# TU-Delft-AI-Energy-Lab/Deep-Statistical-Solver-for-Distribution-System-State-Estimation

Measured on AMD Instinct MI355X. Metric: grid-samples/sec fwd+bwd (WLS loss), CIGRE-14 batch=4096, 1/2/4/8 GPU, higher is better.
Workload: dtype f32 (H->H products as f16x3: two fp16 pieces per operand, 3 fp16 MFMAs per fp32 product, f32 accumulate; edge MLP bf16x6; everything else f32/f64); 1 GPU; CIGRE-14 (15 buses, 14 closed branches) B=4096 graphs/GPU, MPN L=4 H=128 K=2 dropout=0: forward + gsp_wls_edge + backward; graphs_per_gpu=4096, global_batch=4096, parallelism=dp1, ranks_seen=1, arithmetic_route=f16x3, plan_launches=9, clock_ramp_steps_before_warmup=5220, mode=launch plan (dss2_plan_run)

## Files before the change

### deep-statistical-solver-for-distribution-system-state-estimation_amd/csrc/dss2_wgrad16h.hip

```cpp
#include <stdlib.h>

#include "dss2_wgrad_batch.hpp"

namespace dss2 {

#ifdef DSS2_STAMPS
__device__ unsigned long long g_hstamps[512 * 4 * 16];
#define HSTAMP(slot)                                                                                   \
  do {                                                                                                 \
    if (stamp_on) {                                                                                    \
      unsigned long long t_;                                                                           \
      __builtin_amdgcn_sched_barrier(0);                                                               \
      asm volatile("s_memtime %0\n\ts_waitcnt lgkmcnt(0)" : "=s"(t_)::"memory");                      \
      __builtin_amdgcn_sched_barrier(0);                                                               \
      if (lane == 0 && blockIdx.x < 256 && blockIdx.z == 1) g_hstamps[((blockIdx.x * 2 + (blockIdx.y & 1)) * 4 + wv) * 16 + (slot)] = t_; \
    }                                                                                                  \
  } while (0)
#else
#define HSTAMP(slot) do {} while (0)
#endif

constexpr int W16H_TM = 32, W16H_ZC = 64, W16H_XW = 128, W16H_NT = 256, W16H_LDZF = 64, W16H_DMAX = 8;
__device__ __forceinline__ int tph_key(int col) { return (((col >> 3) & 1) << 1) | ((col >> 4) & 1); }
__device__ __forceinline__ int tph_off(int col, int row) { return col * 64 + ((((row >> 3) ^ tph_key(col)) << 4) | ((row & 7) << 1)); }

template <int NCOLS>
__device__ __forceinline__ void store_planes_h(char* img, int off0, const f32x4 v0, const f32x4 v1, int e) {
  const float s = pow2f(e);
#pragma unroll
  for (int q = 0; q < 4; ++q) {
    uint32_t h, l;
    split2_pair(v0[q] * s, v1[q] * s, h, l);
    char* dst = img + off0 + q * 64;
    *reinterpret_cast<uint32_t*>(dst) = h;
    *reinterpret_cast<uint32_t*>(dst + NCOLS * 64) = l;
  }
}

template <int NMAT, bool RS2>
__global__ void __launch_bounds__(W16H_NT, 2) wgrad16h_kernel(const dss2_wgrad_args p, int nibg, const WgradBatch wb, int hb) {
  constexpr int TM = W16H_TM, ZC = W16H_ZC, XW = W16H_XW, NT = W16H_NT, LDZF = W16H_LDZF;
  const float* __restrict__ Gp = wb.n > 0 ? wb.G[blockIdx.z] : p.G;
  const float* __restrict__ Xp = wb.n > 0 ? wb.X[blockIdx.z] : p.X;
  float* __restrict__ slabp = wb.n > 0 ? wb.slab[blockIdx.z] : p.slab;
  const float* __restrict__ rs2 = RS2 ? (wb.n > 0 ? wb.rowscale2[blockIdx.z] : p.rowscale2) : nullptr;
  extern __shared__ __attribute__((aligned(16))) float smem[];
  float* Zf0 = smem;
  float* Zf1 = Zf0 + TM * LDZF;
  char* ZT = reinterpret_cast<char*>(Zf1 + TM * LDZF);
  char* XT = ZT + NMAT * 2 * ZC * 64;
  int2* ell = reinterpret_cast<int2*>(XT + 2 * XW * 64);
  float* mxp = reinterpret_cast<float*>(ell + W16H_DMAX * TM);
  const int D = p.ell_width;

  const int tid = threadIdx.x;
  const int lane = tid & 63, c32 = lane & 31, half = lane >> 5;
  const int wv = __builtin_amdgcn_readfirstlane(tid >> 6);
  const int xb0 = 2 * (wv & 1), obw = wv >> 1;
  const int slice = blockIdx.x, ysl = blockIdx.y;
  const int obg = ysl / nibg, ibg = ysl - obg * nibg;
  const int gcol0 = obg * ZC, xcol0 = ibg * XW;
  const bool x_on[2] = {(xcol0 + xb0 * 32) < p.hin, (xcol0 + (xb0 + 1) * 32) < p.hin};
  const bool in_active = x_on[0] && (gcol0 + obw * 32) < p.hout;

  const int cg = tid & 15, rp = (tid >> 4) ^ ((tid & 1) << 1);
  const int g_off0 = tph_off(4 * cg, 2 * rp);
  const int x_off0[2] = {tph_off(4 * cg, 2 * rp), tph_off(64 + 4 * cg, 2 * rp)};
  const uint32_t g_goff = (uint32_t)((2 * rp) * p.ldg + 4 * cg) * 4u;

  f32x16 acc[2][NMAT];
#pragma unroll
  for (int xb = 0; xb < 2; ++xb)
#pragma unroll
    for (int m = 0; m < NMAT; ++m)
#pragma unroll
      for (int r = 0; r < 16; ++r) acc[xb][m][r] = 0.f;
  f32x4 bsum = {0.f, 0.f, 0.f, 0.f};
  f32x4 bs2[RS2 ? NMAT : 1];
#pragma unroll
  for (int m = 0; m < (RS2 ? NMAT : 1); ++m) bs2[m] = f32x4{0.f, 0.f, 0.f, 0.f};
  int Ex = -100, Eg = -100;

  typedef float f32x3 __attribute__((ext_vector_type(3)));
  f32x4 pg[2], px[4];
  f32x3 prs[RS2 ? 2 : 1];
  int2 pel;
  const uint32_t g_col = (gcol0 + 4 * cg < p.hout) ? (uint32_t)(4 * cg) * 4u : 0u;
  const bool g_ok = gcol0 + 4 * cg < p.hout;
  const uint32_t x_col[2] = {(xcol0 + 4 * cg < p.hin) ? (uint32_t)(4 * cg) * 4u : 0u, (xcol0 + 64 + 4 * cg < p.hin) ? (uint32_t)(64 + 4 * cg) * 4u : 0u};
  const float* __restrict__ rsb = RS2 ? (rs2 ? rs2 : Gp) : nullptr;
  auto load_tile = [&](int tile, int ts, int R) {
    const char* gb = reinterpret_cast<const char*>(Gp + (size_t)ts * p.ldg + gcol0);
    const char* xb = reinterpret_cast<const char*>(Xp + (size_t)ts * p.ldx + xcol0);
#pragma unroll
    for (int u = 0; u < 2; ++u) {
      const int r = 2 * rp + u;
      const int rr = r < R ? r : R - 1;
      pg[u] = *reinterpret_cast<const f32x4*>(gb + (uint32_t)(rr * p.ldg) * 4u + g_col);
      const uint32_t xro = (uint32_t)(rr * p.ldx) * 4u;
#ifdef DSS2_ABLATE_XLOAD
#pragma unroll
      for (int i = 0; i < 2; ++i) px[2 * i + u] = f32x4{1.f, 1.f, 1.f, 1.f};
      (void)xro; (void)xb;
#else
#pragma unroll
      for (int i = 0; i < 2; ++i) px[2 * i + u] = *reinterpret_cast<const f32x4*>(xb + xro + x_col[i]);
#endif
      if constexpr (RS2) prs[u] = *reinterpret_cast<const f32x3*>(rsb + (size_t)(ts + rr) * 4);
    }
    pel = tid < D * TM ? (reinterpret_cast<const int2*>(p.ell_tiles) + (size_t)tile * D * TM)[tid] : make_int2(tid & (TM - 1), 0);
  };
  auto publish_max = [&]() {
    float mx = 0.f, mg = 0.f;
#pragma unroll
    for (int i = 0; i < 4; ++i) mx = absmax4(mx, px[i]);
#pragma unroll
    for (int u = 0; u < 2; ++u) mg = absmax4(mg, pg[u]);
    mx = wave_max(mx); mg = wave_max(mg);
    if (lane == 0) { mxp[wv] = mx; mxp[4 + wv] = mg; }
  };
  auto prop = [&](const float* Zs, float* Zd, char* img, int ez) {
    f32x4 s[2];
#pragma unroll
    for (int u = 0; u < 2; ++u) {
      const int row = 2 * rp + u;
      f32x4 a = {0.f, 0.f, 0.f, 0.f};
      for (int k0 = 0; k0 < D; k0 += 4) {
        int2 en[4];
        f32x4 z[4];
#pragma unroll
        for (int k = 0; k < 4; ++k) en[k] = ell[(k0 + k) * TM + row];
#pragma unroll
        for (int k = 0; k < 4; ++k) z[k] = *reinterpret_cast<const f32x4*>(Zs + en[k].x * LDZF + 4 * cg);
#pragma unroll
        for (int k = 0; k < 4; ++k) {
          const float w = __int_as_float(en[k].y);
#pragma unroll
          for (int q = 0; q < 4; ++q) a[q] = fmaf(w, z[k][q], a[q]);
        }
      }
      s[u] = a;
      if (Zd) *reinterpret_cast<f32x4*>(Zd + row * LDZF + 4 * cg) = a;
    }
    store_planes_h<ZC>(img, g_off0, s[0], s[1], ez);
  };

  int ts = 0, R = 0, ts_n = 0, R_n = 0;
  if (slice < p.ntiles) {
    ts = p.tile_start[slice]; R = p.tile_start[slice + 1] - ts;
    load_tile(slice, ts, R);
    publish_max();
    if (slice + p.n_split < p.ntiles) { ts_n = p.tile_start[slice + p.n_split]; R_n = p.tile_start[slice + p.n_split + 1] - ts_n; }
  }
  __syncthreads();
  for (int tile = slice; tile < p.ntiles; tile += p.n_split) {
    const int next = tile + p.n_split;
#ifdef DSS2_STAMPS
    const bool stamp_on = tile == slice + 2 * p.n_split;
#endif
    HSTAMP(0);
    {
      const f32x4 m0 = *reinterpret_cast<const f32x4*>(mxp), m1 = *reinterpret_cast<const f32x4*>(mxp + 4);
      const int ex = __builtin_amdgcn_readfirstlane(exp_of(fmaxf(fmaxf(m0[0], m0[1]), fmaxf(m0[2], m0[3]))));
      const int eg = __builtin_amdgcn_readfirstlane(exp_of(fmaxf(fmaxf(m1[0], m1[1]), fmaxf(m1[2], m1[3]))));
      const int nx = ex > Ex ? ex : Ex, ng = eg > Eg ? eg : Eg;
      const int d = (nx - Ex) + (ng - Eg);
      if (d != 0) {
#pragma unroll
        for (int xb = 0; xb < 2; ++xb)
#pragma unroll
          for (int m = 0; m < NMAT; ++m)
#pragma unroll
            for (int r = 0; r < 16; ++r) acc[xb][m][r] = ldexpf(acc[xb][m][r], -d);
      }
      Ex = nx; Eg = ng;
    }
    const int sxe = 14 - Ex, sze = 14 - hb - Eg;
    HSTAMP(1);
#pragma unroll
    for (int u = 0; u < 2; ++u)
      if (!(g_ok && 2 * rp + u < R)) pg[u] = f32x4{0.f, 0.f, 0.f, 0.f};
#ifndef DSS2_ABLATE_XSPLIT
#pragma unroll
    for (int i = 0; i < 2; ++i) store_planes_h<XW>(XT, x_off0[i], px[2 * i], px[2 * i + 1], sxe);
#endif
#pragma unroll
    for (int u = 0; u < 2; ++u) *reinterpret_cast<f32x4*>(Zf0 + (2 * rp + u) * LDZF + 4 * cg) = pg[u];
    store_planes_h<ZC>(ZT, g_off0, pg[0], pg[1], sze);
    if (tid < ((D + 3) & ~3) * TM) ell[tid] = pel;
    bsum += pg[0] + pg[1];
    if constexpr (RS2) {
      if (rs2) {
#pragma unroll
        for (int u = 0; u < 2; ++u)
#pragma unroll
          for (int m = 0; m < NMAT; ++m) bs2[m] += pg[u] * prs[u][m];
      }
    }
    HSTAMP(2);
    __syncthreads();
    HSTAMP(3);
    if (next < p.ntiles) load_tile(next, ts_n, R_n);
    HSTAMP(4);
#ifdef DSS2_ABLATE_HOPS
    if (false) {
#else
    if (NMAT > 1) {
#endif
      prop(Zf0, NMAT > 2 ? Zf1 : nullptr, ZT + 2 * ZC * 64, sze);
      HSTAMP(5);
      if (NMAT > 2) {
        __syncthreads();
        HSTAMP(6);
        prop(Zf1, nullptr, ZT + 2 * 2 * ZC * 64, sze);
        HSTAMP(7);
      }
      __syncthreads();
      HSTAMP(8);
    }
#ifdef DSS2_ABLATE_MFMA
    if (false) {
#else
    if (in_active) {
#endif
      const int nsteps = (R + 15) >> 4;
      const int zc = obw * 32 + c32;
      const int zkey = tph_key(zc);
      const int xc0 = xb0 * 32 + c32, xc1 = xc0 + 32;
      const int xkey0 = tph_key(xc0), xkey1 = tph_key(xc1);
      for (int ks = 0; ks < nsteps; ++ks) {
        const int ch = 2 * ks + half;
        f16x8 bh[2], bl[2];
#pragma unroll
        for (int xb = 0; xb < 2; ++xb) {
          const int choff = (xb ? xc1 : xc0) * 64 + ((ch ^ (xb ? xkey1 : xkey0)) << 4);
          bh[xb] = *reinterpret_cast<const f16x8*>(XT + choff);
          bl[xb] = *reinterpret_cast<const f16x8*>(XT + XW * 64 + choff);
        }
        const int zoff = zc * 64 + ((ch ^ zkey) << 4);
#pragma unroll
        for (int m = 0; m < NMAT; ++m) {
          const char* zi = ZT + m * 2 * ZC * 64 + zoff;
          const f16x8 ah = *reinterpret_cast<const f16x8*>(zi);
          const f16x8 al = *reinterpret_cast<const f16x8*>(zi + ZC * 64);
#pragma unroll
          for (int xb = 0; xb < 2; ++xb) {
            if (xb == 1 && !x_on[1]) continue;
            f32x16 c = acc[xb][m];
            c = __builtin_amdgcn_mfma_f32_32x32x16_f16(al, bh[xb], c, 0, 0, 0);
            c = __builtin_amdgcn_mfma_f32_32x32x16_f16(ah, bl[xb], c, 0, 0, 0);
            c = __builtin_amdgcn_mfma_f32_32x32x16_f16(ah, bh[xb], c, 0, 0, 0);
            acc[xb][m] = c;
          }
        }
      }
    }
    HSTAMP(9);
    if (next < p.ntiles) publish_max();
    ts = ts_n; R = R_n;
    if (next + p.n_split < p.ntiles) { ts_n = p.tile_start[next + p.n_split]; R_n = p.tile_start[next + p.n_split + 1] - ts_n; }
    HSTAMP(10);
    __syncthreads();
    HSTAMP(11);
  }

  const size_t stride = (size_t)p.nmat * p.hout * p.hin + p.hout + (rs2 ? (size_t)p.nmat * p.hout : 0);
  float* out = slabp + (size_t)slice * (wb.slab_stride > 0 ? (size_t)wb.slab_stride : stride);
  const int fin = Ex + Eg + hb - 28;
  if (in_active) {
#pragma unroll
    for (int xb = 0; xb < 2; ++xb) {
      const int i = xcol0 + (xb0 + xb) * 32 + c32;
      if (i < p.hin) {
#pragma unroll
        for (int m = 0; m < NMAT; ++m)
#pragma unroll
          for (int r = 0; r < 16; ++r) {
            const int o = gcol0 + obw * 32 + acc_row(r, half);
            if (o < p.hout) out[((size_t)m * p.hout + o) * p.hin + i] = ldexpf(acc[xb][m][r], fin);
          }
      }
    }
  }
  if (ibg == 0) {
    f32x4* red = reinterpret_cast<f32x4*>(smem);
    const int nsum = rs2 ? 1 + NMAT : 1;
    __syncthreads();
    red[tid] = bsum;
    if constexpr (RS2) {
#pragma unroll
      for (int m = 0; m < NMAT; ++m) red[(1 + m) * NT + tid] = bs2[m];
    }
    __syncthreads();
    for (int j = tid; j < nsum * ZC; j += NT) {
      const int which = j / ZC, col = j - which * ZC;
      float s = 0.f;
      for (int r16 = 0; r16 < 16; ++r16) s += red[which * NT + r16 * 16 + (col >> 2)][col & 3];
      const int o = gcol0 + col;
      if (o < p.hout) out[(size_t)p.nmat * p.hout * p.hin + (which == 0 ? 0 : p.hout + (size_t)(which - 1) * p.hout) + o] = s;
    }
  }
}

size_t wgrad16h_lds_bytes(int nmat, int ell_width) {
  const size_t b = 2 * (size_t)W16H_TM * W16H_LDZF * 4 + (size_t)nmat * 2 * W16H_ZC * 64 + 2 * (size_t)W16H_XW * 64 + (size_t)W16H_DMAX * W16H_TM * 8 + 32;
  const size_t red = (size_t)(1 + nmat) * W16H_NT * 16;
  (void)ell_width;
  return b > red ? b : red;
}

bool wgrad16h_covers(const dss2_wgrad_args& a) {
  auto al16 = [](const void* q) { return (reinterpret_cast<uintptr_t>(q) & 15) == 0; };
  return (a.mfma_bf16 & 255) == 2 && a.nrb == 1 && (a.nmat == 2 || a.nmat == 3) && !a.narrow && !a.rowscale && a.ell_tiles && al16(a.G) && al16(a.X) &&
         (a.ldg & 3) == 0 && (a.ldx & 3) == 0 && (!a.rowscale2 || al16(a.rowscale2)) && a.ell_width >= 1 && a.ell_width <= W16H_DMAX &&
         a.hout > 32 && (a.hout & 3) == 0 && (a.hin & 3) == 0;
}

template <int NMAT, bool RS2>
static int launch16h(const dss2_wgrad_args& a, hipStream_t stream, const WgradBatch& wb) {
  static std::atomic<uint32_t> lds_done{0};
  auto kern = wgrad16h_kernel<NMAT, RS2>;
  if (ensure_max_lds(reinterpret_cast<const void*>(kern), lds_done, "wgrad(f16x3, 32 rows)")) return 1;
  const int nobg = (a.hout + W16H_ZC - 1) / W16H_ZC, nibg = (a.hin + W16H_XW - 1) / W16H_XW;
  const int hb = (a.mfma_bf16 >> 8) & 255;
  hipLaunchKernelGGL(kern, dim3(a.n_split, nobg * nibg, wb.n > 0 ? wb.n : 1), dim3(W16H_NT), wgrad16h_lds_bytes(a.nmat, a.ell_width), stream, a, nibg, wb, hb);
  return check_launch("wgrad(f16x3, 32 rows)");
}

int launch_wgrad16h(const dss2_wgrad_args& a, hipStream_t stream, const WgradBatch& wb) {
  bool rs2 = a.rowscale2 != nullptr;
  for (int l = 0; l < wb.n; ++l) {
    if ((reinterpret_cast<uintptr_t>(wb.G[l]) | reinterpret_cast<uintptr_t>(wb.X[l]) | reinterpret_cast<uintptr_t>(wb.rowscale2[l])) & 15) {
      set_error("wgrad(f16x3): layer %d has a misaligned operand", l); return 2;
    }
    rs2 = rs2 || wb.rowscale2[l] != nullptr;
  }
  if (((a.mfma_bf16 >> 8) & 255) > 10) { set_error("wgrad(f16x3): %d headroom bits for the propagation leave no precision", (a.mfma_bf16 >> 8) & 255); return 2; }
  if (a.nmat == 2) return rs2 ? launch16h<2, true>(a, stream, wb) : launch16h<2, false>(a, stream, wb);
  if (a.nmat == 3) return rs2 ? launch16h<3, true>(a, stream, wb) : launch16h<3, false>(a, stream, wb);
  set_error("wgrad(f16x3): unsupported nmat=%d", a.nmat);
  return 2;
}

}

#ifdef DSS2_STAMPS
extern "C" int dss2_debug_read_hstamps(unsigned long long* out, int n) {
  return hipMemcpyFromSymbol(out, HIP_SYMBOL(dss2::g_hstamps), (size_t)n * 8) == hipSuccess ? 0 : 1;
}
#endif
```

### deep-statistical-solver-for-distribution-system-state-estimation_amd/flags.py

```python
import os as _os

EDGE_TILE_KERNELS = _os.environ.get("DSS2_EDGE_TILE", "1") == "1"
CHAIN_LAYERS = _os.environ.get("DSS2_CHAIN", "1") == "1"
WGRAD_BF16 = _os.environ.get("DSS2_WGRAD_BF16", "1") == "1"
CHAIN_GATE_BITS = _os.environ.get("DSS2_CHAIN_GATE_BITS", "1") == "1"
CHAIN_BF16 = _os.environ.get("DSS2_CHAIN_BF16", "1") == "1"
CHAIN_F16 = _os.environ.get("DSS2_CHAIN_F16", "1") == "1"
CHAIN_HEAD = _os.environ.get("DSS2_CHAIN_HEAD", "1") == "1"
CHAIN_HEAD_WGRAD = _os.environ.get("DSS2_CHAIN_HEAD_WGRAD", "1") == "1"
CHAIN_HEAD_FWD = _os.environ.get("DSS2_CHAIN_HEAD_FWD", "1") == "1"
CHAIN_EDGE = _os.environ.get("DSS2_CHAIN_EDGE", "1") == "1"
WGRAD_BATCH = _os.environ.get("DSS2_WGRAD_BATCH", "1") == "1"
STACK_NODE = _os.environ.get("DSS2_STACK_NODE", "1") == "1"
DX_MERGE = _os.environ.get("DSS2_DX_MERGE", "1") == "1"
WGRAD_JOIN_FOLDED = None
FOLD_W2 = _os.environ.get("DSS2_FOLD_W2", "1") == "1"
WGRAD_F16 = _os.environ.get("DSS2_WGRAD_F16", "1") == "1"
WLS_FUSED_FINISH = _os.environ.get("DSS2_WLS_FUSED_FINISH", "0") == "1"
WLS_FUSED_FINISH_SMALL = _os.environ.get("DSS2_WLS_FUSED_FINISH_SMALL", "1") == "1"
WGRAD_TM32 = _os.environ.get("DSS2_WGRAD_TM32", "1") == "1"
WGRAD_TM32_MAX_BYTES = 64 << 20
WGRAD_PER_CU = int(_os.environ.get("DSS2_WGRAD_PER_CU", "2"))
CHAIN_MAX = 8
```

### deep-statistical-solver-for-distribution-system-state-estimation_amd/ops.py

```python
from __future__ import annotations

import ctypes as C
import math
from typing import Optional, Sequence, Tuple

import torch
import torch.nn as nn

from . import _lib
from . import flags as FL
from .topology import Topology


def _static_replay() -> bool:
    from .graphs import plan_recording
    return plan_recording() or torch.cuda.is_current_stream_capturing()


_F32 = torch.float32


def _stream(t: torch.Tensor) -> int:
    return _lib.stream_ptr(t.device)


def _require_gpu(*tensors: torch.Tensor) -> None:
    for t in tensors:
        if t is None:
            continue
        if not t.is_cuda:
            raise RuntimeError("DSS2 HIP path needs GPU tensors (gfx950); there is no CPU fallback")
        if t.is_floating_point() and t.dtype != _F32:
            raise TypeError("DSS2 HIP path computes in fp32; got " + str(t.dtype))


def _rows(t: torch.Tensor) -> Tuple[torch.Tensor, int]:
    if t.dim() != 2:
        raise ValueError("expected a 2-D tensor")
    if t.stride(1) != 1 or (t.size(0) > 1 and t.stride(0) < t.size(1)):
        t = t.contiguous()
    return t, (t.stride(0) if t.size(0) > 1 else t.size(1))


def _ptr(t: Optional[torch.Tensor]) -> Optional[int]:
    return None if t is None else t.data_ptr()


def _round8(k: int) -> int:
    return (k + 7) // 8 * 8


def _round16(k: int) -> int:
    return (k + 15) // 16 * 16


def _ncg(j: int) -> int:
    return (j + 31) // 32


def gemm_prop(topo: Topology, X: torch.Tensor, ldx: int, kreal: int, Bp: torch.Tensor, nmat: int, hout: int,
              Y: torch.Tensor, bias=None, rowscale=None, relu_src=None, dmask=None, add_src=None, add_ld=0,
              relu: bool = False, transposed: bool = False, prop_in: int = 0, narrow_h: int = 0,
              prebias=None, pre_rowscale=None, drop=None, b_format: int = 0) -> None:
    if topo.global_only and (nmat > 1 or prop_in > 0):
        raise NotImplementedError(f"largest connected component has {topo.max_segment} nodes: the fused GEMM + propagation "
                                  "kernels hold a whole graph in LDS (<= 192 nodes); use the MPN / TAGConv modules, which "
                                  "switch to the global-memory propagation path")
    a = _lib.GemmPropArgs()
    if drop is not None and drop[2] > 0:
        a.drop_state, a.drop_id = drop[0].data_ptr(), int(drop[2])
        a.drop_thr, a.drop_scale = _dropout_params(drop[1])
    a.prebias, a.pre_rowscale = _ptr(prebias), _ptr(pre_rowscale)
    a.prop_in, a.narrow_h = prop_in, narrow_h
    a.X, a.ldx, a.kreal, a.kpad = X.data_ptr(), ldx, kreal, (_round16(kreal) if b_format == 1 else _round8(kreal))
    a.b_format = b_format
    a.Bp, a.bias, a.rowscale = Bp.data_ptr(), _ptr(bias), _ptr(rowscale)
    a.relu_src, a.ld_relu = _ptr(relu_src), (relu_src.stride(0) if relu_src is not None else 0)
    a.dmask, a.ld_dmask = _ptr(dmask), (dmask.stride(0) if dmask is not None else 0)
    a.add_src, a.ld_add = _ptr(add_src), add_ld
    a.Y, a.ldy, a.hout, a.ncg = Y.data_ptr(), Y.stride(0), hout, (1 if narrow_h else _ncg(hout))
    a.relu, a.nmat, a.nrb, a.ntiles = int(relu), nmat, topo.nrb, topo.ntiles
    a.tile_start = topo.tile_start.data_ptr()
    if transposed:
        a.rowptr, a.col, a.w, a.max_nnz = topo.rowptrT.data_ptr(), topo.colT.data_ptr(), topo.wT.data_ptr(), topo.max_nnzT
        a.ell_width, a.ell_tiles = topo.ellT, _ptr(topo.ellT_tiles)
    else:
        a.rowptr, a.col, a.w, a.max_nnz = topo.rowptr.data_ptr(), topo.col.data_ptr(), topo.w.data_ptr(), topo.max_nnz
        a.ell_width, a.ell_tiles = topo.ell, _ptr(topo.ell_tiles)
    _lib.check(_lib.lib().dss2_gemm_prop(C.byref(a), _stream(Y)), "dss2_gemm_prop")




def chain_supported(topo: Topology, nmat: int, hid: int, transposed: bool, have16: bool = False) -> bool:
    ell, tiles = (topo.ellT, topo.ellT_tiles) if transposed else (topo.ell, topo.ell_tiles)
    if not FL.CHAIN_LAYERS or tiles is None:
        return False
    return bool(_lib.lib().dss2_gemm_prop_chain_supported(topo.nrb, nmat, hid, hid, ell)) or (
        have16 and chain16_supported(topo, nmat, hid, transposed))


def _single_group_tall_veto(topo: Topology, hid: int) -> bool:
    if hid > 32 or topo.nrb not in (3, 6):
        return False
    m = int(_lib.lib().dss2_chain_sp6_single_group_min_tiles())
    return m < 0 or topo.ntiles < m


def chain_gate_words(topo: Topology, nmat: int, hid: int) -> int:
    if not (FL.CHAIN_LAYERS and FL.CHAIN_BF16 and FL.CHAIN_GATE_BITS) or topo.ell_tiles is None or topo.ellT_tiles is None:
        return 0
    if _single_group_tall_veto(topo, hid):
        return 0
    cache = topo.__dict__.setdefault("_gate_words", {})
    gw = cache.get((nmat, hid))
    if gw is None:
        L = _lib.lib()
        gw = cache[(nmat, hid)] = min(int(L.dss2_gemm_prop_chain_gate_words(topo.nrb, nmat, hid, hid, topo.ell)),
                                      int(L.dss2_gemm_prop_chain_gate_words(topo.nrb, nmat, hid, hid, topo.ellT)))
    return gw


def chain16_supported(topo: Topology, nmat: int, hid: int, transposed: bool) -> bool:
    ell, tiles = (topo.ellT, topo.ellT_tiles) if transposed else (topo.ell, topo.ell_tiles)
    return FL.CHAIN_BF16 and tiles is not None and bool(_lib.lib().dss2_gemm_prop_chain16_supported(topo.nrb, nmat, hid, hid, ell))


def chain_f16_supported(topo: Topology, nmat: int, hid: int) -> bool:
    if not (FL.CHAIN_F16 and FL.CHAIN_BF16 and topo.ell_tiles is not None and topo.ellT_tiles is not None and chain_gate_words(topo, nmat, hid) > 0):
        return False
    L = _lib.lib()
    return bool(L.dss2_gemm_prop_chain_f16_supported(topo.nrb, nmat, hid, hid, topo.ell)) and bool(L.dss2_gemm_prop_chain_f16_supported(topo.nrb, nmat, hid, hid, topo.ellT))


def chain_head_supported(topo: Topology, nmat: int, hid: int, nout: int, transposed: bool) -> bool:
    ell, tiles = (topo.ellT, topo.ellT_tiles) if transposed else (topo.ell, topo.ell_tiles)
    if _single_group_tall_veto(topo, hid):
        return False
    return bool(FL.CHAIN_HEAD) and FL.CHAIN_BF16 and tiles is not None and bool(
        _lib.lib().dss2_gemm_prop_chain_head_supported(topo.nrb, nmat, hid, hid, ell, nout) & (2 if transposed else 1))


def chain_edge_supported(topo: Topology, nmat: int, hid: int, transposed: bool) -> bool:
    if not (FL.CHAIN_EDGE and FL.EDGE_TILE_KERNELS and topo.ell_ent_tiles is not None and topo.ell_tiles is not None and topo.ellT_tiles is not None):
        return False
    ell = topo.ellT if transposed else topo.ell
    return bool(_lib.lib().dss2_gemm_prop_chain_edge_supported(topo.nrb, nmat, hid, hid, ell, topo.ell) & (2 if transposed else 1))


def chain_head_wgrad_supported(topo: Topology, nmat: int, hid: int, nout: int) -> bool:
    return bool(FL.CHAIN_HEAD_WGRAD) and topo.ellT_tiles is not None and bool(
        _lib.lib().dss2_gemm_prop_chain_head_wgrad_supported(topo.nrb, nmat, hid, hid, topo.ellT, nout))


def gemm16_supported(topo: Topology, nmat: int, hid: int, transposed: bool) -> bool:
    ell, tiles, nnz = (topo.ellT, topo.ellT_tiles, topo.max_nnzT) if transposed else (topo.ell, topo.ell_tiles, topo.max_nnz)
    return FL.CHAIN_BF16 and tiles is not None and bool(_lib.lib().dss2_gemm_prop16_supported(topo.nrb, nmat, hid, hid, nnz, ell))


def gemm_prop_chain(topo: Topology, X: Optional[torch.Tensor], hid: int, nmat: int, layers: Sequence[dict], transposed: bool = False,
                    pre_rowscale=None, drop=None, b_format: int = 0, head: Optional[dict] = None) -> None:
    if head is not None and len(layers) > FL.CHAIN_MAX:
        raise ValueError("gemm_prop_chain: a fused head needs the whole chain in one launch")
    if len(layers) > FL.CHAIN_MAX:
        for c0 in range(0, len(layers), FL.CHAIN_MAX):
            gemm_prop_chain(topo, X if c0 == 0 else layers[c0 - 1]["Y"], hid, nmat, layers[c0:c0 + FL.CHAIN_MAX],
                            transposed=transposed, pre_rowscale=pre_rowscale, drop=drop, b_format=b_format)
        return
    a = _lib.GemmPropArgs()
    a.b_format = b_format
    if drop is not None:
        a.drop_state = drop[0].data_ptr()
        a.drop_thr, a.drop_scale = _dropout_params(drop[1])
    dev_t = X if X is not None else layers[-1]["Y"]
    a.X, a.ldx = (X.data_ptr(), X.stride(0)) if X is not None else (0, hid)
    a.kreal, a.kpad = hid, (_round16(hid) if b_format >= 1 else _round8(hid))
    a.hout, a.ncg, a.ldy, a.ld_relu, a.ld_dmask, a.ld_add = hid, _ncg(hid), hid, hid, hid, hid
    a.nmat, a.nrb, a.ntiles = nmat, topo.nrb, topo.ntiles
    a.max_tile_rows = int(getattr(topo, "max_tile_rows", 0) or 0)
    a.tile_start = topo.tile_start.data_ptr()
    a.pre_rowscale = _ptr(pre_rowscale)
    if transposed:
        a.rowptr, a.col, a.w, a.max_nnz = topo.rowptrT.data_ptr(), topo.colT.data_ptr(), topo.wT.data_ptr(), topo.max_nnzT
        a.ell_width, a.ell_tiles = topo.ellT, _ptr(topo.ellT_tiles)
    else:
        a.rowptr, a.col, a.w, a.max_nnz = topo.rowptr.data_ptr(), topo.col.data_ptr(), topo.w.data_ptr(), topo.max_nnz
        a.ell_width, a.ell_tiles = topo.ell, _ptr(topo.ell_tiles)
    tab = (_lib.ChainLayer * len(layers))()
    for d, ly in zip(tab, layers):
        for t_ in (ly.get("Y"), ly.get("relu_src"), ly.get("dmask")):
            if t_ is not None and (t_.stride(0) != hid or t_.stride(1) != 1):
                raise ValueError("gemm_prop_chain: [N, hid] contiguous tensors expected")
        d.Bp, d.Y, d.bias = ly["Bp"].data_ptr(), _ptr(ly.get("Y")), _ptr(ly.get("bias"))
        d.relu_src, d.dmask, d.prebias = _ptr(ly.get("relu_src")), _ptr(ly.get("dmask")), _ptr(ly.get("prebias"))
        d.gate_bits, d.y_bits = _ptr(ly.get("gate_bits")), _ptr(ly.get("y_bits"))
        d.relu = int(bool(ly.get("relu", False)))
        d.drop_id = int(ly.get("drop_id", 0)) if drop is not None else 0
    if head is None:
        _lib.check(_lib.lib().dss2_gemm_prop_chain(C.byref(a), C.addressof(tab), len(layers), _stream(dev_t)), "dss2_gemm_prop_chain")
        return
    hd = _lib.ChainHead()
    for m, w_ in enumerate(head["W"]):
        if w_.stride(0) != hid or w_.stride(1) != 1:
            raise ValueError("gemm_prop_chain: head weights [nout, hid] contiguous expected")
        hd.W[m] = w_.data_ptr()
    hd.nout = int(head["nout"])
    if not transposed:
        hd.mode = 1
        y_ = head["Y"]
        hd.Y, hd.ldy, hd.bias = y_.data_ptr(), y_.stride(0), _ptr(head.get("bias"))
        add_ = head.get("add_src")
        if add_ is not None:
            hd.add_src, hd.ld_add = add_.data_ptr(), int(head["add_ld"])
    else:
        hd.mode = 2
        g_, xo_ = head["G"], head["Xout"]
        hd.G, hd.ldg, hd.Xout, hd.ldxo = g_.data_ptr(), g_.stride(0), xo_.data_ptr(), xo_.stride(0)
        gate_ = head.get("gate")
        if gate_ is not None:
            hd.gate, hd.ld_gate = gate_.data_ptr(), gate_.stride(0)
        hd.drop_id = int(head.get("drop_id", 0)) if drop is not None else 0
        hd.wg_slab = _ptr(head.get("wg_slab"))
        hd.pad = int(head.get("wg_stride", 0))
    edge = head.get("edge")
    if edge is not None:
        e = hd.edge
        e.x, e.ldx, e.ea, e.ldea = edge["x"].data_ptr(), int(edge["ldx"]), edge["ea"].data_ptr(), int(edge["ldea"])
        e.W1, e.b1, e.ell_ent, e.width = edge["W1"].data_ptr(), edge["b1"].data_ptr(), topo.ell_ent_tiles.data_ptr(), topo.ell
        e.S, e.slab = _ptr(edge.get("S")), _ptr(edge.get("slab"))
    _lib.check(_lib.lib().dss2_gemm_prop_chain_head(C.byref(a), C.addressof(tab), len(layers), C.byref(hd), _stream(dev_t)),
               "dss2_gemm_prop_chain_head")


def _wgrad_tiles(topo: Topology, nmat: int, hout: int, hin: int, b16: int):
    if (FL.WGRAD_TM32 and b16 and topo.nrb == 2 and not topo.global_only and nmat in (2, 3) and hout > 32 and 1 <= topo.ellT <= 8
            and (FL.WGRAD_F16 or topo.N * hin * 4 <= FL.WGRAD_TM32_MAX_BYTES)):
        alt = topo.tiles_for(1)
        if alt is not None and alt.ellT_tiles is not None and 1 <= alt.ellT <= 8:
            L_ = _lib.lib()
            if (L_.dss2_wgrad_lds_bytes_ex(1, nmat, hout, hin, alt.max_nnzT, alt.ellT, 1)
                    != L_.dss2_wgrad_lds_bytes_ex(1, nmat, hout, hin, alt.max_nnzT, alt.ellT, 0)):
                return alt
    return topo


def _wgrad_mode(ts, nmat: int, b16: int, hinted: bool = False) -> int:
    if not (b16 and FL.WGRAD_F16 and ts.nrb in (1, 3, 4, 5, 6) and nmat in (2, 3) and ts.ellT_tiles is not None and 1 <= ts.ellT <= 8):
        return b16
    cache = ts.__dict__.setdefault("_f16_gain_bits", {})
    hb = cache.get(nmat)
    if hb is None:
        if hinted or torch.cuda.is_current_stream_capturing():
            gain = float(max(int(ts.ellT), 1))
        else:
            w = ts.ellT_tiles[..., 1].contiguous().view(torch.float32)
            gain = max(float(w.abs().sum(dim=1).max()), 1.0)
        hb = cache[nmat] = max(0, int(math.ceil(math.log2(gain) * (nmat - 1) - 1e-6)))
    return (2 | (hb << 8)) if hb <= 10 else b16


def wgrad(topo: Topology, G: torch.Tensor, hout: int, X: torch.Tensor, hin: int, nmat: int, out_flat: torch.Tensor,
          rowscale=None, rowscale2=None, pending=None, out_len: Optional[int] = None) -> None:
    if topo.global_only and nmat > 1:
        raise NotImplementedError("wgrad with propagation needs LDS-resident graph tiles (graphs of <= 192 nodes)")
    narrow = nmat > 1 and nmat * hout <= 32 and rowscale2 is None
    b16 = int(FL.WGRAD_BF16 and rowscale is None and not narrow)
    ts = _wgrad_tiles(topo, nmat, hout, hin, b16)
    lds = _lib.lib().dss2_wgrad_lds_bytes_ex(ts.nrb, nmat, hout, hin, ts.max_nnzT, ts.ellT, b16)
    per_cu = _wgrad_per_cu(int(lds))
    ys = _lib.lib().dss2_wgrad_y_slices(ts.nrb, nmat, hout, hin, ts.ellT, b16, int(rowscale2 is not None))
    n_split = min(ts.ntiles, max(1, (256 * per_cu) // ys))
    stride = nmat * hout * hin + hout + (nmat * hout if rowscale2 is not None else 0)
    slab = torch.empty(n_split * stride, dtype=_F32, device=G.device)
    a = _lib.WgradArgs()
    a.G, a.ldg, a.hout = G.data_ptr(), G.stride(0), hout
    a.X, a.ldx, a.hin = X.data_ptr(), X.stride(0), hin
    a.rowscale, a.rowscale2 = _ptr(rowscale), _ptr(rowscale2)
    a.slab, a.n_split, a.nmat, a.nrb, a.ntiles = slab.data_ptr(), n_split, nmat, ts.nrb, ts.ntiles
    a.tile_start = ts.tile_start.data_ptr()
    a.rowptrT, a.colT, a.wT, a.max_nnz = topo.rowptrT.data_ptr(), topo.colT.data_ptr(), topo.wT.data_ptr(), ts.max_nnzT
    a.ell_width, a.ell_tiles = ts.ellT, _ptr(ts.ellT_tiles)
    a.narrow, a.mfma_bf16 = int(narrow), (_wgrad_mode(ts, nmat, b16, getattr(topo, "hint", None) is not None) if (not narrow and rowscale is None) else b16)
    st = _stream(G)
    _lib.check(_lib.lib().dss2_wgrad(C.byref(a), st), "dss2_wgrad")
    _reduce(slab, 0, n_split, stride, out_flat, stride if out_len is None else out_len, pending)


def wgrad_batched(topo: Topology, Gs: Sequence[torch.Tensor], hout: int, Xs: Sequence[torch.Tensor], hin: int, nmat: int,
                  out_flat: torch.Tensor, first_rowscale2=None, first_out=None, pending=None) -> None:
    nl = len(Gs)
    ts = _wgrad_tiles(topo, nmat, hout, hin, int(FL.WGRAD_BF16))
    lds = _lib.lib().dss2_wgrad_lds_bytes_ex(ts.nrb, nmat, hout, hin, ts.max_nnzT, ts.ellT, int(FL.WGRAD_BF16))
    per_cu = _wgrad_per_cu(int(lds))
    ys = _lib.lib().dss2_wgrad_y_slices(ts.nrb, nmat, hout, hin, ts.ellT, int(FL.WGRAD_BF16), int(first_rowscale2 is not None))
    mode = _wgrad_mode(ts, nmat, int(FL.WGRAD_BF16), getattr(topo, "hint", None) is not None)
    nz = int(_lib.lib().dss2_wgrad_batched_groups(ts.nrb, hout, hin, mode, nl))
    n_split = min(ts.ntiles, max(1, (256 * per_cu) // (nz * ys)))
    stride = nmat * hout * hin + hout
    lens = [stride + (nmat * hout if (first_rowscale2 is not None and l == 0) else 0) for l in range(nl)]
    total = sum(lens)
    slab = torch.empty(n_split * total, dtype=_F32, device=Gs[0].device)
    a = _lib.WgradArgs()
    a.ldg, a.hout, a.ldx, a.hin = Gs[0].stride(0), hout, Xs[0].stride(0), hin
    for g_, x_ in zip(Gs, Xs):
        if g_.stride(0) != a.ldg or x_.stride(0) != a.ldx or g_.shape != Gs[0].shape or x_.shape != Xs[0].shape:
            raise ValueError("wgrad_batched: layers must share shapes and leading dimensions")
    a.n_split, a.nmat, a.nrb, a.ntiles = n_split, nmat, ts.nrb, ts.ntiles
    a.mfma_bf16 = mode
    a.tile_start = ts.tile_start.data_ptr()
    a.rowptrT, a.colT, a.wT, a.max_nnz = topo.rowptrT.data_ptr(), topo.colT.data_ptr(), topo.wT.data_ptr(), ts.max_nnzT
    a.ell_width, a.ell_tiles = ts.ellT, _ptr(ts.ellT_tiles)
    PtrArr = C.c_void_p * nl
    gs, xs = PtrArr(*[g_.data_ptr() for g_ in Gs]), PtrArr(*[x_.data_ptr() for x_ in Xs])
    offs = [sum(lens[:l]) for l in range(nl)]
    sl = PtrArr(*[slab.data_ptr() + 4 * o for o in offs])
    rs = PtrArr(*[(first_rowscale2.data_ptr() if (first_rowscale2 is not None and l == 0) else None) for l in range(nl)])
    st = _stream(Gs[0])
    L_ = _lib.lib()
    _lib.check(L_.dss2_wgrad_batched(C.byref(a), gs, xs, sl, rs, total, nl, st), "dss2_wgrad_batched")
    if first_rowscale2 is not None:
        _reduce(slab, 0, n_split, total, first_out, lens[0], pending)
        if nl > 1:
            _reduce(slab, lens[0], n_split, total, out_flat, total - lens[0], pending)
    else:
        _reduce(slab, 0, n_split, total, out_flat, total, pending)


def _reduce(slab: torch.Tensor, slab_off: int, n_slabs: int, stride: int, out: torch.Tensor, length: int, pending) -> None:
    if pending is not None:
        pending.append((slab, slab.data_ptr() + 4 * slab_off, n_slabs, stride, out, length))
        return
    _lib.check(_lib.lib().dss2_reduce_slabs(slab.data_ptr() + 4 * slab_off, n_slabs, stride, out.data_ptr(), length,
                                            _stream(slab)), "dss2_reduce_slabs")


def _reduce_descs(chunk):
    descs = (_lib.ReduceDesc * len(chunk))()
    for d, (slab, ptr, n_slabs, stride, out, length) in zip(descs, chunk):
        d.slab, d.out, d.stride, d.len, d.n_slabs = ptr, out.data_ptr(), stride, length, n_slabs
    return descs


def reduce_pending(pending) -> None:
    for c0 in range(0, len(pending), 32):
        chunk = pending[c0:c0 + 32]
        descs = _reduce_descs(chunk)
        _lib.check(_lib.lib().dss2_reduce_slabs_multi(C.addressof(descs), len(chunk), _stream(chunk[0][0])),
                   "dss2_reduce_slabs_multi")
    pending.clear()


def prep_weights(fold_tab, pack_tab, device) -> None:
    t, cnt, mx, _n_dep = pack_tab
    st = _lib.stream_ptr(device)
    if fold_tab is not None:
        ft, fcnt, fmx = fold_tab
        _lib.check(_lib.lib().dss2_small_gemm(ft.data_ptr(), fcnt, fmx, None, st), "dss2_small_gemm")
    _lib.check(_lib.lib().dss2_pack_weights(t.data_ptr(), cnt, mx, st), "dss2_pack_weights")


def finish_weights(pending, rule_tab, base: Optional[torch.Tensor], device) -> None:
    if pending:
        reduce_pending(pending)
    if rule_tab is None:
        return
    rt, rcnt, rmx = rule_tab
    _lib.check(_lib.lib().dss2_small_gemm(rt.data_ptr(), rcnt, rmx, base.data_ptr(), _lib.stream_ptr(device)), "dss2_small_gemm")


def segment_sum(msg: torch.Tensor, rowptr: torch.Tensor, ent: torch.Tensor, n_rows: int) -> torch.Tensor:
    _require_gpu(msg)
    msg, ldm = _rows(msg)
    if ent.dtype != torch.int32:
        ent = ent.to(torch.int32)
    out = torch.empty(n_rows, msg.size(1), dtype=_F32, device=msg.device)
    _lib.check(_lib.lib().dss2_segment_sum(msg.data_ptr(), ldm, rowptr.data_ptr(), ent.data_ptr(), out.data_ptr(),
                                           out.stride(0), n_rows, msg.size(1), _stream(msg)), "dss2_segment_sum")
    return out



def _wgrad_per_cu(lds: int) -> int:
    return max(1, min(FL.WGRAD_PER_CU, (160 * 1024) // max(lds, 1)))


def is_narrow(nmat: int, hout: int) -> bool:
    return nmat > 1 and nmat * hout <= 32


def csr_axpy(topo: Topology, T: torch.Tensor, out: torch.Tensor, h: int, add=None, transposed: bool = False, bias=None,
             relu: bool = False, relu_src=None, add_src=None, add_ld: int = 0, drop=None) -> None:
    a = _lib.CsrAxpyArgs()
    if transposed:
        a.rowptr, a.col, a.w = topo.rowptrT.data_ptr(), topo.colT.data_ptr(), topo.wT.data_ptr()
    else:
        a.rowptr, a.col, a.w = topo.rowptr.data_ptr(), topo.col.data_ptr(), topo.w.data_ptr()
    a.T, a.ldt, a.out, a.ldo = T.data_ptr(), T.stride(0), out.data_ptr(), out.stride(0)
    a.add, a.ld_add = _ptr(add), (add.stride(0) if add is not None else 0)
    a.bias, a.relu = _ptr(bias), int(relu)
    a.relu_src, a.ld_relu = _ptr(relu_src), (relu_src.stride(0) if relu_src is not None else 0)
    a.add_src, a.ld_src = _ptr(add_src), add_ld
    if drop is not None and drop[2] > 0:
        a.drop_state, a.drop_id = drop[0].data_ptr(), int(drop[2])
        a.drop_thr, a.drop_scale = _dropout_params(drop[1])
    a.n_rows, a.h = topo.N, h
    _lib.check(_lib.lib().dss2_csr_axpy(C.byref(a), _stream(out)), "dss2_csr_axpy")


_DROP_PARAMS = {}


def _dropout_params(p: float):
    v = _DROP_PARAMS.get(p)
    if v is None:
        thr, sc = C.c_uint32(), C.c_float()
        _lib.lib().dss2_dropout_params(float(p), C.byref(thr), C.byref(sc))
        v = _DROP_PARAMS[p] = (thr.value, sc.value)
    return v


def dropout_snapshot(mod: nn.Module, device) -> torch.Tensor:
    host_seed = int(torch.empty((), dtype=torch.int64).random_().item())
    st = getattr(mod, "_rng_state", None)
    if st is None or st.device != device:
        st = mod._rng_state = torch.tensor([host_seed ^ 0x5DEECE66D, 0], dtype=torch.int64).to(device)
    snap = torch.empty(2, dtype=torch.int64, device=device)
    capturing = _static_replay()
    _lib.check(_lib.lib().dss2_rng_next(st.data_ptr(), snap.data_ptr(), host_seed, int(not capturing),
                                        _lib.stream_ptr(device)), "dss2_rng_next")
    return snap


def dropout_mask(snapshot: torch.Tensor, p: float, drop_id: int, n_rows: int, h: int) -> torch.Tensor:
    out = torch.empty(n_rows, h, dtype=_F32, device=snapshot.device)
    _lib.check(_lib.lib().dss2_dropout_mask(snapshot.data_ptr(), drop_id, float(p), n_rows, h, out.data_ptr(), h,
                                            _lib.stream_ptr(snapshot.device)), "dss2_dropout_mask")
    return out


def gather_rows(src: torch.Tensor, idx: torch.Tensor) -> torch.Tensor:
    src, lds = _rows(src)
    out = torch.empty(idx.numel(), src.size(1), dtype=_F32, device=src.device)
    _lib.check(_lib.lib().dss2_gather_rows(src.data_ptr(), lds, idx.data_ptr(), out.data_ptr(), out.stride(0) if out.size(0) > 1 else out.size(1),
                                           idx.numel(), src.size(1), _stream(src)), "dss2_gather_rows")
    return out
```

Before: 10.65 million graphs/s.

## Compute wgrad graph-propagation hops with f16x3 MFMA on a dense tile adjacency

Replaces the per-thread sparse ELL gather-FMA propagation in the f16x3 wgrad kernel with a dense 32x32 propagation matrix. Each tile's ELL entries are scattered into LDS as hi/lo fp16 planes, with duplicate indices merged through DPP xor-lane reductions. Each hop then runs as three 16x16x32 f16 MFMAs per block, writing split planes directly. This drops the f32 Z staging buffers and ELL LDS, shrinking LDS. It adds a zeroing pass per tile and depends on the headroom scaling (hb) to keep fp16 precision.

```diff
diff --git a/deep-statistical-solver-for-distribution-system-state-estimation_amd/csrc/dss2_wgrad16h.hip b/deep-statistical-solver-for-distribution-system-state-estimation_amd/csrc/dss2_wgrad16h.hip
--- a/deep-statistical-solver-for-distribution-system-state-estimation_amd/csrc/dss2_wgrad16h.hip
+++ b/deep-statistical-solver-for-distribution-system-state-estimation_amd/csrc/dss2_wgrad16h.hip
@@ -37,7 +37,22 @@
   }
 }
 
-template <int NMAT, bool RS2>
+__device__ __forceinline__ int hop_col(int j, int wv) {
+  const int j2 = (j >> 2) & 1, j3 = (j >> 3) & 1;
+  return (j & 3) + 4 * (wv & 1) + 8 * (j2 ^ j3) + 16 * j3 + 32 * (wv >> 1);
+}
+template <int M>
+__device__ __forceinline__ int xor8(int v) {
+  constexpr int QP[4] = {0xE4, 0xB1, 0x4E, 0x1B};
+  if constexpr (M < 4) return __builtin_amdgcn_update_dpp(0, v, QP[M], 0xf, 0xf, true);
+  else {
+    const int y = __builtin_amdgcn_update_dpp(0, v, 0x141, 0xf, 0xf, true);
+    if constexpr (M == 7) return y;
+    else return __builtin_amdgcn_update_dpp(0, y, QP[7 ^ M], 0xf, 0xf, true);
+  }
+}
+
+template <int NMAT, bool RS2, bool HM>
 __global__ void __launch_bounds__(W16H_NT, 2) wgrad16h_kernel(const dss2_wgrad_args p, int nibg, const WgradBatch wb, int hb) {
   constexpr int TM = W16H_TM, ZC = W16H_ZC, XW = W16H_XW, NT = W16H_NT, LDZF = W16H_LDZF;
   const float* __restrict__ Gp = wb.n > 0 ? wb.G[blockIdx.z] : p.G;
@@ -47,10 +62,11 @@
   extern __shared__ __attribute__((aligned(16))) float smem[];
   float* Zf0 = smem;
   float* Zf1 = Zf0 + TM * LDZF;
-  char* ZT = reinterpret_cast<char*>(Zf1 + TM * LDZF);
+  char* ZT = reinterpret_cast<char*>(smem) + (HM ? 0 : 2 * TM * LDZF * 4);
   char* XT = ZT + NMAT * 2 * ZC * 64;
   int2* ell = reinterpret_cast<int2*>(XT + 2 * XW * 64);
-  float* mxp = reinterpret_cast<float*>(ell + W16H_DMAX * TM);
+  char* PT = XT + 2 * XW * 64;
+  float* mxp = reinterpret_cast<float*>(XT + 2 * XW * 64 + (HM ? 2 * TM * 64 : W16H_DMAX * TM * 8));
   const int D = p.ell_width;
 
   const int tid = threadIdx.x;
@@ -66,7 +82,13 @@
   const int cg = tid & 15, rp = (tid >> 4) ^ ((tid & 1) << 1);
   const int g_off0 = tph_off(4 * cg, 2 * rp);
   const int x_off0[2] = {tph_off(4 * cg, 2 * rp), tph_off(64 + 4 * cg, 2 * rp)};
-  const uint32_t g_goff = (uint32_t)((2 * rp) * p.ldg + 4 * cg) * 4u;
+  const int pk = tid & 7, prow = tid >> 3;
+  const int pkc = pk < D ? pk : D - 1;
+  const int hj = lane & 15, hg = lane >> 4;
+  const int hc = hop_col(hj, wv);
+  const int hop_b = hc * 64 + ((hg ^ tph_key(hc)) << 4);
+  const int hop_a[2] = {tph_off(hj, 8 * hg), tph_off(16 + hj, 8 * hg)};
+  const int hop_d[2] = {tph_off(hc, 4 * hg), tph_off(hc, 16 + 4 * hg)};
 
   f32x16 acc[2][NMAT];
 #pragma unroll
@@ -108,7 +130,53 @@
 #endif
       if constexpr (RS2) prs[u] = *reinterpret_cast<const f32x3*>(rsb + (size_t)(ts + rr) * 4);
     }
-    pel = tid < D * TM ? (reinterpret_cast<const int2*>(p.ell_tiles) + (size_t)tile * D * TM)[tid] : make_int2(tid & (TM - 1), 0);
+    if constexpr (HM) pel = (reinterpret_cast<const int2*>(p.ell_tiles) + (size_t)tile * D * TM)[pkc * TM + prow];
+    else pel = tid < D * TM ? (reinterpret_cast<const int2*>(p.ell_tiles) + (size_t)tile * D * TM)[tid] : make_int2(tid & (TM - 1), 0);
+  };
+  auto scatter_p = [&]() {
+    const float w = pk < D ? __int_as_float(pel.y) : 0.f;
+    const int idx = w != 0.f ? (pel.x & (TM - 1)) : TM + pk;
+    const int wi = __float_as_int(w);
+    bool s1 = xor8<1>(idx) == idx, s2 = xor8<2>(idx) == idx, s3 = xor8<3>(idx) == idx;
+    bool s4 = false, s5 = false, s6 = false, s7 = false;
+    if (D > 4) { s4 = xor8<4>(idx) == idx; s5 = xor8<5>(idx) == idx; s6 = xor8<6>(idx) == idx; s7 = xor8<7>(idx) == idx; }
+    float tot = w;
+    bool lose = false;
+    if (__builtin_amdgcn_ballot_w64(s1 || s2 || s3 || s4 || s5 || s6 || s7) != 0) {
+      tot += s1 ? __int_as_float(xor8<1>(wi)) : 0.f; lose = lose || (s1 && (pk ^ 1) < pk);
+      tot += s2 ? __int_as_float(xor8<2>(wi)) : 0.f; lose = lose || (s2 && (pk ^ 2) < pk);
+      tot += s3 ? __int_as_float(xor8<3>(wi)) : 0.f; lose = lose || (s3 && (pk ^ 3) < pk);
+      if (D > 4) {
+        tot += s4 ? __int_as_float(xor8<4>(wi)) : 0.f; lose = lose || (s4 && (pk ^ 4) < pk);
+        tot += s5 ? __int_as_float(xor8<5>(wi)) : 0.f; lose = lose || (s5 && (pk ^ 5) < pk);
+        tot += s6 ? __int_as_float(xor8<6>(wi)) : 0.f; lose = lose || (s6 && (pk ^ 6) < pk);
+        tot += s7 ? __int_as_float(xor8<7>(wi)) : 0.f; lose = lose || (s7 && (pk ^ 7) < pk);
+      }
+    }
+    if (!lose && tot != 0.f) {
+      uint32_t h, l;
+      split2_pair(tot * pow2f(14 - hb), 0.f, h, l);
+      char* dst = PT + tph_off(prow, idx & (TM - 1));
+      *reinterpret_cast<uint16_t*>(dst) = (uint16_t)h;
+      *reinterpret_cast<uint16_t*>(dst + TM * 64) = (uint16_t)l;
+    }
+  };
+  auto hop = [&](const char* src, char* dst) {
+    const f16x8 zh = *reinterpret_cast<const f16x8*>(src + hop_b), zl = *reinterpret_cast<const f16x8*>(src + ZC * 64 + hop_b);
+    const float s = pow2f(hb - 14);
+#pragma unroll
+    for (int rb = 0; rb < 2; ++rb) {
+      const f16x8 ph = *reinterpret_cast<const f16x8*>(PT + hop_a[rb]), pl = *reinterpret_cast<const f16x8*>(PT + TM * 64 + hop_a[rb]);
+      f32x4 c = {0.f, 0.f, 0.f, 0.f};
+      c = __builtin_amdgcn_mfma_f32_16x16x32_f16(pl, zh, c, 0, 0, 0);
+      c = __builtin_amdgcn_mfma_f32_16x16x32_f16(ph, zl, c, 0, 0, 0);
+      c = __builtin_amdgcn_mfma_f32_16x16x32_f16(ph, zh, c, 0, 0, 0);
+      uint2 h, l;
+      split2_pair(c[0] * s, c[1] * s, h.x, l.x);
+      split2_pair(c[2] * s, c[3] * s, h.y, l.y);
+      *reinterpret_cast<uint2*>(dst + hop_d[rb]) = h;
+      *reinterpret_cast<uint2*>(dst + ZC * 64 + hop_d[rb]) = l;
+    }
   };
   auto publish_max = [&]() {
     float mx = 0.f, mg = 0.f;
@@ -152,6 +220,7 @@
     publish_max();
     if (slice + p.n_split < p.ntiles) { ts_n = p.tile_start[slice + p.n_split]; R_n = p.tile_start[slice + p.n_split + 1] - ts_n; }
   }
+  if constexpr (HM) *reinterpret_cast<f32x4*>(PT + tid * 16) = f32x4{0.f, 0.f, 0.f, 0.f};
   __syncthreads();
   for (int tile = slice; tile < p.ntiles; tile += p.n_split) {
     const int next = tile + p.n_split;
@@ -184,10 +253,13 @@
 #pragma unroll
     for (int i = 0; i < 2; ++i) store_planes_h<XW>(XT, x_off0[i], px[2 * i], px[2 * i + 1], sxe);
 #endif
-#pragma unroll
-    for (int u = 0; u < 2; ++u) *reinterpret_cast<f32x4*>(Zf0 + (2 * rp + u) * LDZF + 4 * cg) = pg[u];
+    if constexpr (!HM) {
+#pragma unroll
+      for (int u = 0; u < 2; ++u) *reinterpret_cast<f32x4*>(Zf0 + (2 * rp + u) * LDZF + 4 * cg) = pg[u];
+    }
     store_planes_h<ZC>(ZT, g_off0, pg[0], pg[1], sze);
-    if (tid < ((D + 3) & ~3) * TM) ell[tid] = pel;
+    if constexpr (HM) scatter_p();
+    else if (tid < ((D + 3) & ~3) * TM) ell[tid] = pel;
     bsum += pg[0] + pg[1];
     if constexpr (RS2) {
       if (rs2) {
@@ -207,16 +279,19 @@
 #else
     if (NMAT > 1) {
 #endif
-      prop(Zf0, NMAT > 2 ? Zf1 : nullptr, ZT + 2 * ZC * 64, sze);
+      if constexpr (HM) hop(ZT, ZT + 2 * ZC * 64);
+      else prop(Zf0, NMAT > 2 ? Zf1 : nullptr, ZT + 2 * ZC * 64, sze);
       HSTAMP(5);
       if (NMAT > 2) {
         __syncthreads();
         HSTAMP(6);
-        prop(Zf1, nullptr, ZT + 2 * 2 * ZC * 64, sze);
+        if constexpr (HM) hop(ZT + 2 * ZC * 64, ZT + 2 * 2 * ZC * 64);
+        else prop(Zf1, nullptr, ZT + 2 * 2 * ZC * 64, sze);
         HSTAMP(7);
       }
       __syncthreads();
       HSTAMP(8);
+      if constexpr (HM) *reinterpret_cast<f32x4*>(PT + tid * 16) = f32x4{0.f, 0.f, 0.f, 0.f};
     }
 #ifdef DSS2_ABLATE_MFMA
     if (false) {
@@ -302,8 +377,9 @@
   }
 }
 
-size_t wgrad16h_lds_bytes(int nmat, int ell_width) {
-  const size_t b = 2 * (size_t)W16H_TM * W16H_LDZF * 4 + (size_t)nmat * 2 * W16H_ZC * 64 + 2 * (size_t)W16H_XW * 64 + (size_t)W16H_DMAX * W16H_TM * 8 + 32;
+size_t wgrad16h_lds_bytes(int nmat, int ell_width, bool hops_mfma) {
+  const size_t planes = (size_t)nmat * 2 * W16H_ZC * 64 + 2 * (size_t)W16H_XW * 64;
+  const size_t b = hops_mfma ? planes + 2 * (size_t)W16H_TM * 64 + 32 : 2 * (size_t)W16H_TM * W16H_LDZF * 4 + planes + (size_t)W16H_DMAX * W16H_TM * 8 + 32;
   const size_t red = (size_t)(1 + nmat) * W16H_NT * 16;
   (void)ell_width;
   return b > red ? b : red;
@@ -316,14 +392,14 @@
          a.hout > 32 && (a.hout & 3) == 0 && (a.hin & 3) == 0;
 }
 
-template <int NMAT, bool RS2>
+template <int NMAT, bool RS2, bool HM>
 static int launch16h(const dss2_wgrad_args& a, hipStream_t stream, const WgradBatch& wb) {
   static std::atomic<uint32_t> lds_done{0};
-  auto kern = wgrad16h_kernel<NMAT, RS2>;
+  auto kern = wgrad16h_kernel<NMAT, RS2, HM>;
   if (ensure_max_lds(reinterpret_cast<const void*>(kern), lds_done, "wgrad(f16x3, 32 rows)")) return 1;
   const int nobg = (a.hout + W16H_ZC - 1) / W16H_ZC, nibg = (a.hin + W16H_XW - 1) / W16H_XW;
   const int hb = (a.mfma_bf16 >> 8) & 255;
-  hipLaunchKernelGGL(kern, dim3(a.n_split, nobg * nibg, wb.n > 0 ? wb.n : 1), dim3(W16H_NT), wgrad16h_lds_bytes(a.nmat, a.ell_width), stream, a, nibg, wb, hb);
+  hipLaunchKernelGGL(kern, dim3(a.n_split, nobg * nibg, wb.n > 0 ? wb.n : 1), dim3(W16H_NT), wgrad16h_lds_bytes(a.nmat, a.ell_width, HM), stream, a, nibg, wb, hb);
   return check_launch("wgrad(f16x3, 32 rows)");
 }
 
@@ -336,8 +412,11 @@
     rs2 = rs2 || wb.rowscale2[l] != nullptr;
   }
   if (((a.mfma_bf16 >> 8) & 255) > 10) { set_error("wgrad(f16x3): %d headroom bits for the propagation leave no precision", (a.mfma_bf16 >> 8) & 255); return 2; }
-  if (a.nmat == 2) return rs2 ? launch16h<2, true>(a, stream, wb) : launch16h<2, false>(a, stream, wb);
-  if (a.nmat == 3) return rs2 ? launch16h<3, true>(a, stream, wb) : launch16h<3, false>(a, stream, wb);
+  const bool hm = !((a.mfma_bf16 >> 16) & 1);
+  if (a.nmat == 2) return rs2 ? (hm ? launch16h<2, true, true>(a, stream, wb) : launch16h<2, true, false>(a, stream, wb))
+                              : (hm ? launch16h<2, false, true>(a, stream, wb) : launch16h<2, false, false>(a, stream, wb));
+  if (a.nmat == 3) return rs2 ? (hm ? launch16h<3, true, true>(a, stream, wb) : launch16h<3, true, false>(a, stream, wb))
+                              : (hm ? launch16h<3, false, true>(a, stream, wb) : launch16h<3, false, false>(a, stream, wb));
   set_error("wgrad(f16x3): unsupported nmat=%d", a.nmat);
   return 2;
 }
diff --git a/deep-statistical-solver-for-distribution-system-state-estimation_amd/flags.py b/deep-statistical-solver-for-distribution-system-state-estimation_amd/flags.py
--- a/deep-statistical-solver-for-distribution-system-state-estimation_amd/flags.py
+++ b/deep-statistical-solver-for-distribution-system-state-estimation_amd/flags.py
@@ -16,6 +16,7 @@
 WGRAD_JOIN_FOLDED = None
 FOLD_W2 = _os.environ.get("DSS2_FOLD_W2", "1") == "1"
 WGRAD_F16 = _os.environ.get("DSS2_WGRAD_F16", "1") == "1"
+WGRAD_HOPS_MFMA = _os.environ.get("DSS2_WGRAD_HOPS_MFMA", "1") == "1"
 WLS_FUSED_FINISH = _os.environ.get("DSS2_WLS_FUSED_FINISH", "0") == "1"
 WLS_FUSED_FINISH_SMALL = _os.environ.get("DSS2_WLS_FUSED_FINISH_SMALL", "1") == "1"
 WGRAD_TM32 = _os.environ.get("DSS2_WGRAD_TM32", "1") == "1"
diff --git a/deep-statistical-solver-for-distribution-system-state-estimation_amd/ops.py b/deep-statistical-solver-for-distribution-system-state-estimation_amd/ops.py
--- a/deep-statistical-solver-for-distribution-system-state-estimation_amd/ops.py
+++ b/deep-statistical-solver-for-distribution-system-state-estimation_amd/ops.py
@@ -256,7 +256,7 @@
             w = ts.ellT_tiles[..., 1].contiguous().view(torch.float32)
             gain = max(float(w.abs().sum(dim=1).max()), 1.0)
         hb = cache[nmat] = max(0, int(math.ceil(math.log2(gain) * (nmat - 1) - 1e-6)))
-    return (2 | (hb << 8)) if hb <= 10 else b16
+    return (2 | (hb << 8) | (0 if FL.WGRAD_HOPS_MFMA else 1 << 16)) if hb <= 10 else b16
 
 
 def wgrad(topo: Topology, G: torch.Tensor, hout: int, X: torch.Tensor, hin: int, nmat: int, out_flat: torch.Tensor,
```

Measured after the change: 10.92 million graphs/s (median of 6 runs). +2.5%, better.
